# timfpark/heatmap

Hardware: AMD Instinct MI355X
Metric: points binned/sec (whole node, zooms 0-18) + % HBM roofline at 1/2/4/8 GPU (higher is better)
Workload: dtype f64

## Files before the change

heatmap_amd/csrc/hm_api.cpp:

```cpp
#include <hip/hip_runtime.h>
#include <stdio.h>
#include <stdlib.h>
#include <string.h>

#include <math.h>

#include <algorithm>
#include <chrono>
#include <vector>

#include "hm_genkey.h"
#include "hm_ctx.h"

namespace {

struct Level {
    int zc;
    int dbits;
    uint32_t nparents;
    uint64_t nchildren;
    uint32_t count = 0;
    uint32_t items = 0;
    bool out16 = false;
};
// ... 82 lines not shown
    case HM_E_WIDE: return "a routed count needs 64 bits (route again with count_bytes = 8)";
    case HM_E_HIP: return "HIP runtime error";
    case HM_E_NOMEM: return "device allocation failed";
    default: return "unknown status";
    }
}

int hm_ctx_create(hm_ctx** out, int device, void* stream)
{
    if (!out) return HM_E_ARG;
    *out = nullptr;
    int n = 0;
    if (hipGetDeviceCount(&n) != hipSuccess || n <= device || device < 0) {
        (void)hipGetLastError();
        fprintf(stderr, "heatmap_amd: no HIP device %d (found %d); there is no CPU fallback\n", device, n);
        return HM_E_HIP;
    }
    HIPCHK(hipSetDevice(device));
    hm_ctx* c = new hm_ctx();
    c->device = device;
    c->stream = (hipStream_t)stream;
    c->bufs.resize(B_COUNT);
    for (int i = 0; i < HM_NEV; i++) c->ev[i] = nullptr;
    c->spread_min_keys = HM_SPREAD_MIN_KEYS;
    if (const char* e = getenv("HM_SPREAD_MIN_KEYS")) c->spread_min_keys = atof(e);
    c->spread_min_cold = HM_SPREAD_MIN_COLD;
    if (const char* e = getenv("HM_SPREAD_MIN_COLD")) c->spread_min_cold = atof(e);
    c->rs_big_min = HM_RS_BIG;
    if (const char* e = getenv("HM_RS_BIG_MIN")) c->rs_big_min = (uint64_t)atoll(e);
    if (const char* e = getenv("HM_HOT")) c->hot = atoi(e);
    if (const char* e = getenv("HM_HOT_MID")) c->hot_mid = atoi(e);
    if (const char* e = getenv("HM_HOT_INV_SHARE")) c->hot_inv_share = atof(e);
    if (const char* e = getenv("HM_HOT_MIN_KEYS")) c->hot_min_keys = atof(e);
    if (const char* e = getenv("HM_RUN_SHARD_BITS")) c->run_shard_bits = atoi(e);
    if (const char* e = getenv("HM_SAMPLE_LOG2")) c->sample_log2 = std::min(30, std::max(8, atoi(e)));
    if (const char* e = getenv("HM_DEBUG_L1")) c->debug_l1 = atoi(e);
    if (const char* e = getenv("HM_STAGE_TIMING")) c->stage_timing = atoi(e);
    if (const char* e = getenv("HM_CONTIG")) c->contig = atoi(e);
    if (const char* e = getenv("HM_TA_MIN")) c->ta_min = (uint32_t)std::max(1024, std::min((int)HM_TA, atoi(e)));
    if (const char* e = getenv("HM_TA_ITEMS")) c->ta_items = (uint32_t)std::max(1, atoi(e));
    int st = HM_OK;
    if (hipMalloc(&c->state, ST_COUNT * sizeof(unsigned long long)) != hipSuccess) {
        c->state = nullptr;
        st = HM_E_NOMEM;
    } else if (hipHostMalloc(&c->host_state, 4 * ST_COUNT * sizeof(unsigned long long)) != hipSuccess) {
        c->host_state = nullptr;
        st = HM_E_NOMEM;
    } else if (hipHostMalloc(&c->host_aux, (2 + 2 * HM_L1_SHARDS) * HM_D1 * sizeof(uint32_t)) != hipSuccess) {
        c->host_aux = nullptr;
        st = HM_E_NOMEM;
    }
    for (int i = 0; i < HM_NEV && st == HM_OK; i++)
        if (hipEventCreate(&c->ev[i]) != hipSuccess) {
            c->ev[i] = nullptr;
            st = HM_E_HIP;
        }
    if (st != HM_OK) {
        (void)hipGetLastError();
        hm_ctx_destroy(c);
        return st;
    }
    *out = c;
    return HM_OK;
}

int hm_ctx_set_stream(hm_ctx* c, void* stream)
// ... 9 lines not shown
    double prev;
    if (!strcmp(name, "HM_SPREAD_MIN_KEYS")) {
        prev = c->spread_min_keys;
        c->spread_min_keys = value;
    } else if (!strcmp(name, "HM_SPREAD_MIN_COLD")) {
        prev = c->spread_min_cold;
        c->spread_min_cold = value;
    } else if (!strcmp(name, "HM_CONTIG")) {
        prev = c->contig;
        c->contig = value != 0;
    } else if (!strcmp(name, "HM_STAGE_TIMING")) {
        prev = c->stage_timing;
        c->stage_timing = value != 0;
    } else if (!strcmp(name, "HM_SAMPLE_LOG2")) {
        if (!(value >= 8 && value <= 30)) return HM_E_ARG;
        prev = c->sample_log2;
        c->sample_log2 = (int)value;
    } else if (!strcmp(name, "HM_RS_BIG_MIN")) {
        prev = (double)c->rs_big_min;
        c->rs_big_min = (uint64_t)(value < 0 ? 0 : value);
    } else if (!strcmp(name, "HM_HOT")) {
        prev = c->hot;
        c->hot = value != 0;
    } else if (!strcmp(name, "HM_HOT_MID")) {
        prev = c->hot_mid;
        c->hot_mid = value != 0;
    } else if (!strcmp(name, "HM_HOT_INV_SHARE")) {
        if (!(value >= 1)) return HM_E_ARG;
        prev = c->hot_inv_share;
        c->hot_inv_share = value;
    } else if (!strcmp(name, "HM_HOT_MIN_KEYS")) {
        prev = c->hot_min_keys;
        c->hot_min_keys = value;
    } else if (!strcmp(name, "HM_RUN_SHARD_BITS")) {
        if (value > 5) return HM_E_ARG;
        prev = c->run_shard_bits;
        c->run_shard_bits = value < 0 ? -1 : (int)value;
    } else if (!strcmp(name, "HM_TA_MIN")) {
        const uint32_t v = (value >= 1024 && value <= (double)HM_TA) ? (uint32_t)value : 0u;
        if (!v || (double)v != value || (v & (v - 1))) return HM_E_ARG;
        prev = c->ta_min;
        c->ta_min = v;
    } else if (!strcmp(name, "HM_TA_ITEMS")) {
        if (!(value >= 1 && value <= 4294967295.0)) return HM_E_ARG;
        prev = c->ta_items;
        c->ta_items = (uint32_t)value;
    } else {
        return HM_E_ARG;
    }
    if (old) *old = prev;
    return HM_OK;
}

int hm_ctx_destroy(hm_ctx* c)
{
    if (!c) return HM_OK;
    (void)hipSetDevice(c->device);
    for (auto& b : c->bufs)
        if (b.p) (void)hipFree(b.p);
    if (c->state) (void)hipFree(c->state);
    if (c->host_state) (void)hipHostFree(c->host_state);
    if (c->host_aux) (void)hipHostFree(c->host_aux);
    for (int i = 0; i < HM_NEV; i++)
        if (c->ev[i]) (void)hipEventDestroy(c->ev[i]);
    delete c;
    return HM_OK;
// ... 3 lines not shown
{
    if (!c) return HM_E_ARG;
    if (index) *index = c->last_err_index;
    if (kind) *kind = c->last_err_kind;
    return HM_OK;
}

int hm_last_stats(hm_ctx* c, int64_t* slow_points, double* stage_us, int n_stages)
{
    if (!c) return HM_E_ARG;
    if (slow_points) *slow_points = c->last_slow;
    for (int i = 0; i < n_stages && i < 9; i++) stage_us[i] = c->stage_us[i];
    if (n_stages > 7) stage_us[7] = (double)c->last_levels;
    return HM_OK;
}

}

void ctx_copy_tuning(hm_ctx* d, const hm_ctx* c)
{
    d->spread_min_keys = c->spread_min_keys;
    d->spread_min_cold = c->spread_min_cold;
    d->sample_log2 = c->sample_log2;
    d->debug_l1 = c->debug_l1;
    d->stage_timing = c->stage_timing;
    d->contig = c->contig;
    d->ta_min = c->ta_min;
    d->ta_items = c->ta_items;
    d->rs_big_min = c->rs_big_min;
    d->hot = c->hot;
    d->hot_mid = c->hot_mid;
    d->hot_inv_share = c->hot_inv_share;
    d->hot_min_keys = c->hot_min_keys;
    d->run_shard_bits = c->run_shard_bits;
}

static int reset_state(hm_ctx* ctx)
{
    HIPCHK(hipMemsetAsync(ctx->state, 0, ST_COUNT * sizeof(unsigned long long), ctx->stream));
    HIPCHK(hipMemsetAsync(ctx->state + ST_ERR, 0xFF, sizeof(unsigned long long), ctx->stream));
    return HM_OK;
}

static int read_state(hm_ctx* ctx)
{
    HIPCHK(hipMemcpyAsync(ctx->host_state, ctx->state, ST_COUNT * sizeof(unsigned long long), hipMemcpyDeviceToHost,
                          ctx->stream));
    HIPCHK(hm_sync(ctx->stream));
    return HM_OK;
}

static int take_error(hm_ctx* ctx)
{
    const unsigned long long e = ctx->host_state[ST_ERR];
    ctx->last_slow = (int64_t)ctx->host_state[ST_SLOW];
    if (e == ~0ull) {
        ctx->last_err_index = -1;
        ctx->last_err_kind = HM_OK;
        return HM_OK;
    }
    ctx->last_err_index = (int64_t)(e >> 8);
    ctx->last_err_kind = (int)(e & 0xFF);
    return ctx->last_err_kind;
}

extern "C" int hm_project(hm_ctx* ctx, const double* lat, const double* lon, int64_t n, int zoom, int64_t* row,
// ... 465 lines not shown
    hand.slot_k ^= 1;
    return HM_OK;
}

int CountCall::level1()
{
    int st;
    if ((st = begin_level(0))) return st;
    Level1Work w;
    if ((st = level1_setup(w))) return st;
    if ((st = level1_size(w))) return st;
    if ((st = level1_bucket_args(w))) return st;
    if ((st = level1_run(w))) return st;
    return level1_finish(w);
}

int CountCall::level1_setup(Level1Work& w)
{
    const Level& V = lv[0];
    HmFill f1;
    memset(&f1, 0, sizeof(f1));
    hm_fill_add(f1, ctx->state + 1, 0, (ST_COUNT - 1) * sizeof(unsigned long long));
    hm_fill_add(f1, ctx->state + ST_ERR, 0xFF, sizeof(unsigned long long));
    static_assert(ST_ERR == 0, "error word first");
    w.F = 1 << V.dbits;
    uint32_t* fill;
    ENSURE(B_L1_FILL, FS * 4, fill);
    ENSURE(B_L1_RBASE, FS * 4, w.rbase);
    ENSURE(B_L1_RCAP, FS * 4, w.rcap);
    ENSURE(B_L1_HIST, HM_D1 * 4, w.hist);
    ENSURE(B_L1_SMASK, HM_D1, w.smask);
    uint32_t* const hist = w.hist;
    uint4* l1slot = nullptr;
    if (!from_tiles) ENSURE(B_L1_SLOT, (size_t)FS * sizeof(uint4), l1slot);
    hot_mid = ctx->hot && ctx->hot_mid && L == 3 && zs[1] <= 11 && zs[0] == HM_Z1 && n > 0 && V.dbits == 2 * HM_Z1;
    hot_on = hot_mid || (ctx->hot && L == 2 && zb <= 11 && zs[0] == HM_Z1 && n > 0 && V.dbits == 2 * HM_Z1);
    hz = hot_mid ? zs[1] : zb;
    uint32_t* redo_idx = nullptr;
    w.redo_rows = w.redo_cols = nullptr;
    if (!from_tiles) {
        ENSURE(B_REDO_IDX, redo_cap * sizeof(uint32_t), redo_idx);
        ENSURE(B_REDO_ROWS, redo_cap * sizeof(int64_t), w.redo_rows);
        ENSURE(B_REDO_COLS, redo_cap * sizeof(int64_t), w.redo_cols);
    }
    HmPart1Args& a = w.a;
    memset(&a, 0, sizeof(a));
    a.lat = lat;
    a.lon = lon;
    a.rows_in = rows;
    a.cols_in = cols;
    a.keep = keep;
    a.n = n;
    a.Z = Z;
    a.dbits = V.dbits;
    a.restbits = 2 * (Z - zs[0]);
    a.fill = fill;
    a.rbase = w.rbase;
    a.rcap = w.rcap;
    a.smask = w.smask;
    a.l1slot = l1slot;
    a.overflow = ctx->state + ST_OVERFLOW;
    a.err_word = ctx->state + ST_ERR;
    a.x = xl;
    a.slow_count = ctx->state + ST_SLOW;
    a.redo_idx = redo_idx;
    a.redo_count = ctx->state + ST_REDO;
    a.redo_cap = redo_cap;
    const int slog = n < (1ll << 24) ? std::min(ctx->sample_log2, 16) : ctx->sample_log2;
    const uint64_t stride = w.stride = std::max<uint64_t>(1, (uint64_t)n >> slog);
    hm_fill_add(f1, hist, 0, HM_D1 * 4);
    hm_fill_add(f1, fill, 0, FS * 4);
    uint32_t* hot_counts = nullptr;
    uint32_t* hot_tiles = nullptr;
    uint32_t* hot_hash = nullptr;
    uint8_t* hot_parent = nullptr;
    uint32_t* hot_n = (uint32_t*)(ctx->state + ST_NHOT);
    if (hot_on) {
        ENSURE(B_HOT_COUNTS, (4ull << (2 * hz)), hot_counts);
        ENSURE(B_HOT, (HM_MAX_HOT + HM_HOT_SLOTS + 2 * HM_HOT_CAND + 1) * 4, hot_tiles);
        ENSURE(B_HOT_PARENT, HM_MAX_F1, hot_parent);
        hot_hash = hot_tiles + HM_MAX_HOT;
        hm_fill_add(f1, hot_counts, 0, 4ull << (2 * hz));
        hm_fill_add(f1, hot_hash + HM_HOT_SLOTS + 2 * HM_HOT_CAND, 0, 4);
        hm_fill_add(f1, hot_parent, 0, HM_MAX_F1);
        a.hot_z = hz;
        a.hot_bytes = hot_mid ? 4 : 2;
        a.hot_hash = hot_hash;
        a.hot_n = hot_n;
    } else {
        a.hot_z = -1;
    }
    hm_launch_fill(s, f1);
    if (n > 0) hm_launch_sample_digits(s, a, stride, hist, hot_counts);
// ... 1362 lines not shown
```

heatmap_amd/csrc/hm_ctx.h:

```cpp
#ifndef HM_CTX_H
#define HM_CTX_H

#include <hip/hip_runtime.h>

#include <vector>

#include "../../include/heatmap_amd.h"
#include "hm_pipeline.h"

#define HM_INTERNAL __attribute__((visibility("hidden")))

struct HM_INTERNAL Buf {
    void* p = nullptr;
    size_t cap = 0;
};

#define HM_NEV 12

#define HM_FALLBACK (-1)

struct hm_ctx {
    int device = 0;
    hipStream_t stream = nullptr;
    std::vector<Buf> bufs;
    unsigned long long* state = nullptr;
    unsigned long long* host_state = nullptr;
    int last_levels = 0;
    uint32_t* host_aux = nullptr;
    int64_t last_err_index = -1;
    int last_err_kind = 0;
    int64_t last_slow = 0;
    double stage_us[9] = {0};
    hipEvent_t ev[HM_NEV];
    double spread_min_keys = 0;
    double spread_min_cold = 0;
    int sample_log2 = 18;
    int debug_l1 = 0;
    int stage_timing = 1;
    int contig = 1;
    uint32_t ta_min = 16384;
    uint32_t ta_items = 128;
    uint64_t* tail_keys = nullptr;
    const unsigned long long* tail_state = nullptr;
    int tail_cb = 0;
    int tail_done = 0;
    uint64_t rs_big_min = 0;
    int hot = 1;
    int hot_mid = 1;
    double hot_inv_share = 4096;
    double hot_min_keys = 65536;
    int run_shard_bits = -1;
};

enum {
    ST_ERR = 0,
    ST_XCOUNT = 1,
    ST_SLOW = 2,
    ST_CURSOR = 3,
    ST_NSLOTS = 4,
    ST_REDO = 5,
    ST_REDO_OUT = 6,
    ST_XCURSOR = 7,
    ST_OVERFLOW = 8,
    ST_NHOT = 9,
    ST_L1TOTAL = 10,
    ST_LTOT = 12,
    ST_COUNT = 16
};

enum {
    B_KEYS_A, B_KEYS_B, B_RUNS_SH, B_FLAT_A, B_FLAT_B, B_EXCL_A, B_EXCL_B, B_CNT, B_SHOFF, B_NR, B_NRUNS,
    B_NKEYS, B_KEYBASE, B_VALS, B_PREFIX, B_PARTIAL, B_TOTAL, B_ROOT, B_REDO_IDX, B_REDO_ROWS, B_REDO_COLS,
    B_RUNBASE0,
    B_BK0 = B_RUNBASE0 + HM_MAX_LEVELS,
    B_CHILD0 = B_BK0 + HM_MAX_LEVELS * 8,
    B_TOT0 = B_CHILD0 + HM_MAX_LEVELS,
    B_SLOTS = B_TOT0 + HM_MAX_LEVELS + 1,
    B_SLOTBKT, B_GSLOTS, B_SPCODES, B_DESC0,
    B_X_ROW = B_DESC0 + HM_MAX_LEVELS, B_X_COL, B_X_IDX, B_GEN_KA, B_GEN_KB, B_GEN_FLAG, B_GEN_IDX, B_GEN_C,
    B_GEN_KHA, B_GEN_KHB, B_GEN_HIST, B_GEN_ORAND, B_GL_GRP,
    B_L1_FILL, B_L1_RBASE, B_L1_RCAP, B_L1_HIST, B_L1_SMASK,
    B_RT_CNT, B_RT_OFF, B_MG_TABLE, B_MG_STATE, B_SEG, B_RS_BIG,
    B_HOT, B_HOT_COUNTS, B_HOT_PARENT, B_D2B, B_MB_CNT, B_MB_OFF, B_MB_KEYS, B_MB_COUNTS, B_MB_CNT2, B_MB_OFF2,
// ... 43 lines not shown
```

heatmap_amd/csrc/hm_kernels.hip:

```cpp
#include <hip/hip_runtime.h>
#include "hm_genkey.h"
#include "hm_device.h"
#include "hm_project.h"
#include "hm_pipeline.h"
#define HM_STAMP_MODES(m) ((m) >= 1 && (m) <= 4)
#include "hm_stamps.h"
#include "hm_runs.h"

#define HM_YTAB_N (HM_YTAB_ROWS * HM_YTAB_STRIDE)
__constant__ double c_ytab[HM_YTAB_N] = HM_YTAB_INIT;

__device__ __forceinline__ void hm_load_ytab(double* tab)
{
    for (int i = threadIdx.x; i < HM_YTAB_N; i += blockDim.x) tab[i] = c_ytab[i];
}


__global__ __launch_bounds__(256) void k_project(const double* __restrict__ lat, const double* __restrict__ lon,
                                                 int64_t n, int zoom, int64_t* __restrict__ row,
                                                 int64_t* __restrict__ col, uint8_t* __restrict__ status,
                                                 unsigned long long* err_word, unsigned long long* slow_count)
{
    __shared__ double tab[HM_YTAB_N];
    hm_load_ytab(tab);
// ... 42 lines not shown
    return x;
}

#define HM_PIN16(x)                                                                                                   \
    "+v"(x[0]), "+v"(x[1]), "+v"(x[2]), "+v"(x[3]), "+v"(x[4]), "+v"(x[5]), "+v"(x[6]), "+v"(x[7]), "+v"(x[8]),       \
        "+v"(x[9]), "+v"(x[10]), "+v"(x[11]), "+v"(x[12]), "+v"(x[13]), "+v"(x[14]), "+v"(x[15])
template <int N>
__device__ __forceinline__ void hm_pin_all(uint32_t (&x)[N])
{
    if constexpr (N == 16) {
        asm volatile("" : HM_PIN16(x));
    } else {
#pragma unroll
        for (int k = 0; k < N; k++) asm volatile("" : "+v"(x[k]));
    }
}
template <int N>
__device__ __forceinline__ void hm_pin_all(uint32_t (&x)[N], uint32_t& y)
{
    if constexpr (N == 16) {
        asm volatile("" : HM_PIN16(x), "+v"(y));
    } else {
#pragma unroll
        for (int k = 0; k < N; k++) asm volatile("" : "+v"(x[k]));
        asm volatile("" : "+v"(y));
    }
}

typedef double hm_d2v __attribute__((ext_vector_type(2)));
__device__ __forceinline__ double2 hm_stream_load2(const double2* p)
{
    const hm_d2v v = __builtin_nontemporal_load((const hm_d2v*)p);
    return make_double2(v.x, v.y);
}

__device__ __forceinline__ uint32_t hm_hot_find(const uint2* tab, uint32_t rs, uint32_t cs)
{
    const uint2 e = tab[hm_hot_bucket(rs, cs)];
    const uint32_t tk = rs << HM_HOT_TAG;
    return min(e.x ^ tk, e.y ^ tk);
}


template <typename OutT, int MODE, bool FULL>
__global__ __launch_bounds__(HM_P1_THREADS, HM_P1_WAVES) void k_project_partition(HmPart1Args a)
{
    __shared__ uint32_t cur[HM_D1 + 64];
    __shared__ __attribute__((aligned(16))) OutT stage[HM_T1 + 64];
    __shared__ __attribute__((aligned(8))) uint16_t sdig[HM_T1 + 64];
    __shared__ unsigned long long scr[HM_P1_THREADS / 64 + 1];
    __shared__ double tab[HM_YTAB_N];
    constexpr bool HSEP = sizeof(OutT) * HM_T1 < HM_HOT_SLOTS * 4;
    constexpr bool RSEP = sizeof(uint16_t) * HM_T1 < HM_D1 * sizeof(uint2);
    __shared__ __attribute__((aligned(16))) uint32_t hsep[HSEP ? HM_HOT_SLOTS : 4];
    __shared__ __attribute__((aligned(8))) uint2 rsep[RSEP ? HM_D1 : 1];
    static_assert(sizeof(double) * HM_YTAB_N >= HM_D1 * 4, "dbase lives in the polynomial table");
    uint4* const hsh4 = HSEP ? (uint4*)hsep : (uint4*)stage;
    uint32_t* const dbase = (uint32_t*)tab;
    uint2* const rinfo = RSEP ? rsep : (uint2*)sdig;
    constexpr bool FROM_TILES = MODE == 1;
    const int tid = threadIdx.x;
    const int F = 1 << a.dbits;
    const uint32_t H = a.hot_z >= 0 ? *a.hot_n : 0u;
    const int64_t base = (a.tile0 + (int64_t)blockIdx.x) * HM_T1;
    const int64_t n = (FROM_TILES && a.n_dev) ? min((int64_t)*a.n_dev, a.n) : a.n;
    if (base >= n) return;
// ... 305 lines not shown
#endif
#define HM_L1_SLOTS (HM_MAX_HOT + HM_MAX_F1)
#define HM_L1_CW 1600
static_assert(HM_L1_CW >= HM_L1_SLOTS + 64 && HM_L1_CW % 64 == 0, "count and delta words pair as read2st64");
static_assert(HM_L1_SLOTS % HM_P1_THREADS == 0, "slots per thread");

#ifndef HM_L1_WAVES
#define HM_L1_WAVES 4
#endif

__device__ __forceinline__ uint32_t hm_l1_slot_digit(uint32_t sl, int wd)
{
    if (sl < HM_MAX_HOT) return HM_MAX_F1 + sl;
    const uint32_t u = sl - HM_MAX_HOT, m = (1u << wd) - 1u;
    return HM_SKEW_CUR ? ((u & ~m) | ((u - ((u >> wd) << 3)) & m)) : u;
}
__device__ __forceinline__ bool hm_l1_slot_live(uint32_t sl, uint32_t H, uint32_t F)
{
    return sl < HM_MAX_HOT ? sl < H : (sl - HM_MAX_HOT) < F;
}

__global__ __launch_bounds__(256) void k_l1_slots(HmPart1Args a, uint4* __restrict__ tab)
{
    const uint32_t sl = blockIdx.x * 256u + threadIdx.x, b = blockIdx.y;
    if (sl >= HM_D1) return;
    const uint32_t H = a.hot_z >= 0 ? min(*a.hot_n, (uint32_t)HM_MAX_HOT) : 0u;
    uint4 e = make_uint4(0u, 0u, 0u, 0u);
    if (hm_l1_slot_live(sl, H, 1u << a.dbits)) {
        const uint32_t d = hm_l1_slot_digit(sl, a.dbits >> 1);
        const uint32_t i = hm_l1i(d, a.smask[d] != 0 ? b : 0u);
        e = make_uint4(a.rbase[i], a.rcap[i], i, 0u);
    }
    tab[b * HM_D1 + sl] = e;
}

void hm_launch_l1_slots(hipStream_t s, const HmPart1Args& a)
{
    static_assert(HM_D1 == HM_MAX_HOT + HM_MAX_F1, "the table's rows are k_l1_fast's slots");
    hipLaunchKernelGGL(k_l1_slots, dim3((HM_D1 + 255) / 256, HM_L1_SHARDS), dim3(256), 0, s, a, (uint4*)a.l1slot);
}
template <typename OutT, bool KEEP>
__global__ __launch_bounds__(HM_P1_THREADS) __attribute__((amdgpu_waves_per_eu(HM_L1_WAVES, HM_L1_WAVES))) void
k_l1_fast(HmPart1Args a)
{
    __shared__ __attribute__((aligned(16))) uint2 ent[HM_T1 + 64];
    __shared__ uint32_t cw[2 * HM_L1_CW];
    __shared__ uint32_t scr[HM_P1_THREADS / 64 + 1];
    __shared__ uint32_t s_over;
    constexpr int YROWS = HM_YTAB_ROWS + 1;
    constexpr int YN = YROWS * HM_YTAB_STRIDE;
    static_assert(sizeof(double) * YN <= 16384 && HM_HOT_SLOTS * 4 <= 16384, "tables fit the stage");
    double* const tab = (double*)ent;
    uint2* const hot2 = (uint2*)((char*)ent + 16384);
    const int tid = threadIdx.x;
    const uint32_t H = a.hot_z >= 0 ? *a.hot_n : 0u;
    const int64_t base = (a.tile0 + (int64_t)blockIdx.x) * HM_T1;
    HM_STAMP_M(4, 0);
    const double scale = hm_exp2i(a.Z);
    const double nscale = -scale, hscale = 0.5 * scale;
    const double kz = HM_INV360 * scale;
    const double c180 = 180.0 * kz;
    const double ghalf = 0.5 - HM_Y_EPS * scale;
    const double ghalf2 = 0.5 - scale * 0x1p-49;
    constexpr int PERD = HM_L1_SLOTS / HM_P1_THREADS;
    const int wd = a.dbits >> 1;
    uint32_t kp[HM_P1_PPT / 2];
    if (KEEP) {
        const uint16_t* kp2 = (const uint16_t*)(a.keep + base);
#pragma unroll
        for (int k = 0; k < HM_P1_PPT / 2; k++) kp[k] = kp2[k * HM_P1_THREADS + tid];
    } else {
#pragma unroll
        for (int k = 0; k < HM_P1_PPT / 2; k++) kp[k] = 0x0101;
    }
    __builtin_amdgcn_sched_barrier(0);
    constexpr int TPT = (YN + HM_P1_THREADS - 1) / HM_P1_THREADS;
    double tv[TPT];
#pragma unroll
    for (int q = 0; q < TPT; q++) {
        const int i = q * HM_P1_THREADS + tid;
        tv[q] = i >= HM_YTAB_N ? __builtin_nan("") : c_ytab[i];
    }
    uint4 st[PERD];
    {
        const uint4* const row = a.l1slot + (blockIdx.x & (HM_L1_SHARDS - 1)) * HM_L1_SLOTS;
#pragma unroll
        for (int q = 0; q < PERD; q++) st[q] = row[q * HM_P1_THREADS + tid];
    }
    constexpr int HV = HM_HOT_SLOTS / 4 / HM_P1_THREADS;
    uint4 hv[HV];
    static_assert(HM_HOT_SLOTS <= HM_D1 * HM_L1_SHARDS, "the stand-in array holds a hot table's bytes");
    const uint4* const hsrc = H ? (const uint4*)a.hot_hash : (const uint4*)a.rbase;
#pragma unroll
    for (int j = 0; j < HV; j++) {
        const uint4 v = hsrc[j * HM_P1_THREADS + tid];
        hv[j] = make_uint4(v.x, v.y, v.z, v.w);
    }
    __builtin_amdgcn_sched_barrier(0);
    double2 la[HM_P1_PPT / 2], lo[HM_P1_PPT / 2];
    {
        const double2* lat2 = (const double2*)(a.lat + base);
        const double2* lon2 = (const double2*)(a.lon + base);
#pragma unroll
        for (int k = 0; k < HM_P1_PPT / 2; k++) {
            la[k] = hm_stream_load2(lat2 + k * HM_P1_THREADS + tid);
            lo[k] = hm_stream_load2(lon2 + k * HM_P1_THREADS + tid);
        }
    }
    for (int i = tid; i < HM_L1_CW; i += HM_P1_THREADS) cw[i] = 0;
    if (tid == 0) s_over = 0;
    if (H) {
#pragma unroll
        for (int j = 0; j < HV; j++) ((uint4*)hot2)[j * HM_P1_THREADS + tid] = hv[j];
    }
#pragma unroll
    for (int q = 0; q < TPT; q++) {
        const int i = q * HM_P1_THREADS + tid;
        if (i < YN) tab[i] = tv[q];
    }
    hm_lds_barrier();
    HM_STAMP_M(4, 1);
    const int hb = a.restbits >> 1;
    const uint32_t lowm = (1u << hb) - 1u;
    const uint32_t keym = (uint32_t)((1ull << (2 * hb)) - 1ull);
    const uint32_t wm = (1u << wd) - 1u;
    const int hs = a.hot_z >= 0 ? a.Z - a.hot_z : 0;
    const uint32_t dummy = HM_L1_SLOTS + (uint32_t)hm_lane();
    uint32_t slot[HM_P1_PPT], key[HM_P1_PPT];
    uint32_t redo = 0;
#pragma unroll
    for (int k = 0; k < HM_P1_PPT; k++) {
        const double pa = (k & 1) ? la[k >> 1].y : la[k >> 1].x;
        const double po = (k & 1) ? lo[k >> 1].y : lo[k >> 1].x;
        uint32_t r, c;
        const bool ok = hm_project_l1(pa, po, nscale, hscale, kz, c180, ghalf, ghalf2, tab, &r, &c);
        const bool kept = ((kp[k >> 1] >> (8 * (k & 1))) & 0xFFu) != 0;
        redo |= (uint32_t)!ok << k;
        const uint32_t rd = r >> hb, cd = c >> hb;
        const uint32_t rdw = (rd << wd) + HM_MAX_HOT;
        uint32_t sl = HM_SKEW_CUR ? (((cd + (rd << 3)) & wm) | rdw) : (cd | rdw);
        if (H) sl = min(hm_hot_find(hot2, r >> hs, c >> hs), sl);
        key[k] = ((r << hb) | (c & lowm)) & keym;
        slot[k] = (ok & kept) ? sl : dummy;
        asm volatile("" : "+v"(slot[k]), "+v"(key[k]));
        __builtin_amdgcn_sched_barrier(0);
    }
    HM_STAMP_M(4, 2);
    if (__builtin_amdgcn_ballot_w64(redo != 0)) {
#pragma unroll
        for (int k = 0; k < HM_P1_PPT; k++) {
            const bool rd = (redo >> k) & 1u;
            const uint64_t m = __builtin_amdgcn_ballot_w64(rd);
            if (m) {
                uint64_t b = 0;
                if (hm_lane() == __ffsll((unsigned long long)m) - 1) b = atomicAdd(a.redo_count, (unsigned long long)__popcll(m));
                b = __shfl(b, __ffsll((unsigned long long)m) - 1, 64);
                const uint64_t q = b + hm_mbcnt(m);
                if (rd && q < a.redo_cap)
                    a.redo_idx[q] = (uint32_t)(base + 2 * ((int64_t)(k >> 1) * HM_P1_THREADS + tid) + (k & 1));
            }
        }
        const uint32_t ws = hm_wave_sum((uint32_t)__popc(redo));
        if (hm_lane() == 0 && ws) atomicAdd(a.slow_count, (unsigned long long)ws);
    }
    uint32_t rank[HM_P1_PPT];
    uint32_t merged = 0;
#pragma unroll
    for (int k = 0; k < HM_P1_PPT; k++) {
        const uint32_t k0 = __builtin_amdgcn_readfirstlane(slot[k]);
        const uint64_t m = __builtin_amdgcn_ballot_w64(slot[k] == k0);
        const uint32_t pm = (uint32_t)__builtin_popcount((uint32_t)m) + (uint32_t)__builtin_popcount((uint32_t)(m >> 32));
        uint32_t idx = slot[k], inc = 1u;
        if (pm >= HM_L1_MERGE_MIN) {
            merged |= 1u << k;
            const bool in = (m >> hm_lane()) & 1ull;
            idx = (in && hm_lane() != 0) ? dummy : idx;
            inc = hm_lane() == 0 ? pm : inc;
        }
        rank[k] = atomicAdd(&cw[idx], inc);
    }
    if (merged) {
#pragma unroll
        for (int k = 0; k < HM_P1_PPT; k++)
            if ((merged >> k) & 1u) {
                const uint32_t k0 = __builtin_amdgcn_readfirstlane(slot[k]);
                const uint64_t m = __builtin_amdgcn_ballot_w64(slot[k] == k0);
                const uint32_t r0 = __builtin_amdgcn_readfirstlane(rank[k]);
                if ((m >> hm_lane()) & 1ull) rank[k] = r0 + hm_mbcnt(m);
            }
    }
    hm_lds_barrier();
    HM_STAMP_M(4, 3);
    uint32_t cnt[PERD], gpos[PERD];
#pragma unroll
    for (int q = 0; q < PERD; q++) {
        const uint32_t sl = q * HM_P1_THREADS + tid;
        cnt[q] = cw[sl];
        gpos[q] = 0;
        if (cnt[q]) gpos[q] = atomicAdd(&a.fill[st[q].z], cnt[q]);
    }
    constexpr int QH = HM_MAX_HOT / HM_P1_THREADS;
    static_assert(HM_MAX_HOT % HM_P1_THREADS == 0 && QH >= 1 && QH < PERD, "slots q < QH are the hot tiles");
    uint32_t csum = 0, hsum = 0;
#pragma unroll
    for (int q = 0; q < PERD; q++) (q < QH ? hsum : csum) += cnt[q];
    uint32_t tot2;
    const uint32_t pre = hm_block_excl_scan<HM_P1_THREADS, true>(csum | (hsum << 16), scr, &tot2);
    const uint32_t C = tot2 & 0xFFFFu, total = C + (tot2 >> 16);
    uint32_t offq[PERD];
    {
        uint32_t oc = pre & 0xFFFFu, oh = C + (pre >> 16);
#pragma unroll
        for (int q = 0; q < PERD; q++) {
            offq[q] = q < QH ? oh : oc;
            (q < QH ? oh : oc) += cnt[q];
        }
    }
    bool over = false;
    auto deltas = [&]() {
#pragma unroll
        for (int q = 0; q < PERD; q++) {
            const uint32_t sl = q * HM_P1_THREADS + tid;
            const uint32_t rc = st[q].y, rb = st[q].x;
            const bool fits = (uint64_t)gpos[q] + cnt[q] <= (uint64_t)rc;
            over |= cnt[q] && !fits;
            cw[HM_L1_CW + sl] = (fits ? rb + gpos[q] : 0xFFF00000u) - offq[q];
        }
        if (over) {
            atomicOr(a.overflow, 1ull);
            s_over = 1;
        }
    };
#pragma unroll
    for (int q = 0; q < PERD; q++) {
        const uint32_t sl = q * HM_P1_THREADS + tid;
        cw[sl] = offq[q];
    }
    hm_lds_barrier();
    HM_STAMP_M(4, 4);
#pragma unroll
    for (int k = 0; k < HM_P1_PPT; k++) {
        const uint32_t o = cw[slot[k]];
        const uint32_t pos = slot[k] < HM_L1_SLOTS ? o + rank[k] : HM_T1 + (uint32_t)hm_lane();
        ent[pos] = make_uint2(key[k], slot[k]);
    }
    deltas();
    hm_lds_barrier();
    HM_STAMP_M(4, 5);
    char* const outb = (char*)a.keys_out;
    char* const houtb = (char*)a.keys_hot;
    const uint32_t hm = (1u << hs) - 1u;
    auto put_cold = [&](uint2 e) { *(OutT*)(outb + (uint64_t)e.y * sizeof(OutT)) = (OutT)e.x; };
    const bool hot32 = a.hot_bytes == 4;
    auto put_hot = [&](uint2 e) {
        const uint32_t hk = (((e.x >> hb) & hm) << hs) | (e.x & hm);
        if (hot32) *(uint32_t*)(houtb + (uint64_t)e.y * 4u) = hk;
        else *(uint16_t*)(houtb + (uint64_t)e.y * 2u) = (uint16_t)hk;
    };
    uint2 e[HM_P1_PPT];
    uint32_t sov;
    uint32_t dl[HM_P1_PPT];
#pragma unroll
    for (int j = 0; j < HM_P1_PPT; j++) {
        e[j] = ent[j * HM_P1_THREADS + tid];
        dl[j] = e[j].y;
    }
    hm_pin_all(dl);
#pragma unroll
    for (int j = 0; j < HM_P1_PPT; j++) dl[j] = cw[HM_L1_CW + min(dl[j], (uint32_t)(HM_L1_CW - 1))];
    sov = s_over;
    hm_pin_all(dl, sov);
    sov = __builtin_amdgcn_readfirstlane(sov);
#pragma unroll
    for (int j = 0; j < HM_P1_PPT; j++) e[j].y = dl[j] + (uint32_t)(j * HM_P1_THREADS + tid);
    const uint32_t wofs = (uint32_t)tid & ~63u;
    if (!sov) {
#pragma unroll
        for (int j = 0; j < HM_P1_PPT; j++) {
            const uint32_t wb = __builtin_amdgcn_readfirstlane(j * HM_P1_THREADS + wofs);
            const uint32_t i = j * HM_P1_THREADS + tid;
            if (wb + 64 <= C) {
                put_cold(e[j]);
            } else if (wb >= C && wb + 64 <= total) {
                put_hot(e[j]);
            } else if (wb < total) {
                if (i < C) put_cold(e[j]);
                else if (i < total) put_hot(e[j]);
            }
        }
    } else {
#pragma unroll
        for (int j = 0; j < HM_P1_PPT; j++) {
            const uint32_t i = j * HM_P1_THREADS + tid;
            if (i < total && e[j].y < 0xFFF00000u) {
                if (i < C) put_cold(e[j]);
                else put_hot(e[j]);
            }
        }
    }
    HM_STAMP_M(4, 6);
}

#define HM_SAMPLE_HSLOTS 4096
template <bool FROM_TILES, bool HOT>
__global__ __launch_bounds__(256) void k_sample_digits(HmPart1Args a, uint64_t stride_pts, uint32_t* hist,
                                                       uint32_t* hot_counts)
{
    __shared__ uint32_t h[HM_MAX_F1 + 64];
    __shared__ double tab[HM_YTAB_N];
    __shared__ uint32_t hk[HOT ? HM_SAMPLE_HSLOTS : 1], hc[HOT ? HM_SAMPLE_HSLOTS : 1];
    const int F = 1 << a.dbits;
    for (int i = threadIdx.x; i < F; i += 256) h[i] = 0;
    if (HOT)
        for (int i = threadIdx.x; i < HM_SAMPLE_HSLOTS; i += 256) {
            hk[i] = HM_HOT_EMPTY;
            hc[i] = 0;
        }
    if (!FROM_TILES) hm_load_ytab(tab);
    __syncthreads();
    uint32_t hlost = 0;
    const double scale = hm_exp2i(a.Z);
    const double kz = HM_INV360 * scale;
    const uint32_t lim = 1u << a.Z;
    const int hb = a.restbits >> 1, wd = a.dbits >> 1;
    const uint64_t m = (uint64_t)(a.n + stride_pts - 1) / stride_pts;
    const uint64_t m_up = (m + 63) & ~63ull;
    const uint64_t step = (uint64_t)gridDim.x * 256;
    for (uint64_t j = (uint64_t)blockIdx.x * 256 + threadIdx.x; j < m_up; j += step) {
        const uint64_t i = j * stride_pts;
// ... 1601 lines not shown
```

heatmap_amd/csrc/hm_pipeline.h:

```cpp
#pragma once
#include <hip/hip_runtime.h>
#include <stdint.h>

#include "hm_top_select.h"

#ifndef HM_P1_THREADS
#define HM_P1_THREADS 512
#endif
#ifndef HM_P1_PPT
#define HM_P1_PPT 16
#endif
#define HM_T1 (HM_P1_THREADS * HM_P1_PPT)
#ifndef HM_P1_GROUP
#define HM_P1_GROUP 4
#endif
#ifndef HM_P1_ILP
#define HM_P1_ILP 1
#endif
#ifndef HM_P1_WAVES
#define HM_P1_WAVES 1
#endif
#define HM_L1_SHARDS 8
#ifndef HM_L1_SHARD_TILES
#define HM_L1_SHARD_TILES 16
#endif
#define HM_L1_ZERO_SAMPLES 24
#define HM_Z1 5
#define HM_MAX_F1 1024
#ifndef HM_MAX_HOT
#define HM_MAX_HOT 512
#endif
#define HM_HOT_LIMIT HM_MAX_HOT
#define HM_D1 (HM_MAX_F1 + HM_MAX_HOT)
#define HM_HOT_WAYS 2
#define HM_HOT_SLOTS 4096
#define HM_HOT_BUCKETS (HM_HOT_SLOTS / HM_HOT_WAYS)
#define HM_HOT_BBITS 11
#define HM_HOT_TAG 16
#define HM_HOT_MULT 0x9E3779u
#define HM_HOT_CAND 4096
#define HM_HOT_EMPTY 0xFFFFFFFFu
static_assert(HM_MAX_HOT <= 1024 && (HM_MAX_HOT & 255) == 0, "hot tiles");
__host__ __device__ inline uint32_t hm_hot_bucket(uint32_t rs, uint32_t cs)
{
#if defined(__HIP_DEVICE_COMPILE__)
    return (__umul24(rs, HM_HOT_MULT) + cs) & (HM_HOT_BUCKETS - 1u);
#else
    return (rs * HM_HOT_MULT + cs) & (HM_HOT_BUCKETS - 1u);
#endif
}
static_assert(HM_HOT_MULT < (1u << 24), "24-bit hash multiplier");
static_assert(HM_HOT_BUCKETS == 1 << HM_HOT_BBITS, "hot-tile table");
__host__ __device__ inline uint32_t hm_l1i(uint32_t d, uint32_t sh) { return sh * HM_D1 + d; }
#ifndef HM_PN_THREADS
#define HM_PN_THREADS 1024
#endif
#ifndef HM_TN
#define HM_TN 8192
#endif
#ifndef HM_FR_THREADS
#define HM_FR_THREADS 1024
#endif
#ifndef HM_FR_GROUP
#define HM_FR_GROUP 4
#endif
#ifndef HM_LEVEL_ZOOMS
#define HM_LEVEL_ZOOMS 6
#endif
#define HM_MAX_FN 4096
#define HM_MAX_SHARDS 32
#ifndef HM_RUN_SHARD_BITS
#define HM_RUN_SHARD_BITS 4
#endif
#define HM_AG_THREADS 1024
#define HM_AG_CELLS 16384
#define HM_AG_LG 7
#ifndef HM_TA
#define HM_TA (1u << 18)
#endif
#ifndef HM_SP_MAX
#define HM_SP_MAX 512
#endif
#ifndef HM_SPW_MAX
#define HM_SPW_MAX HM_SP_MAX
#endif
#ifndef HM_SPW_SPLIT
// ... 77 lines not shown
    uint64_t cap;
    unsigned long long* count;
};

struct HmCompactOut {
    uint32_t* nkeys;
    uint32_t* nruns;
    uint32_t* rbase;
    uint32_t* keybase;
    uint32_t* item_begin;
    uint32_t* digit;
    uint64_t* coord;
};

struct HmPart1Args {
    const double* lat;
    const double* lon;
    const int64_t* rows_in;
    const int64_t* cols_in;
    const uint8_t* keep;
    int64_t n;
    int64_t tile0;
    const unsigned long long* n_dev;
    int Z, dbits, restbits;
    uint32_t* redo_idx;
    unsigned long long* redo_count;
    uint64_t redo_cap;
    void* keys_out;
    uint32_t* fill;
    const uint32_t* rbase;
    const uint32_t* rcap;
    const uint8_t* smask;
    const uint4* l1slot;
    unsigned long long* overflow;
    unsigned long long* err_word;
    HmExotic x;
    unsigned long long* slow_count;
    int hot_z;
    int hot_bytes;
    void* keys_hot;
    const uint32_t* hot_hash;
    const uint32_t* hot_n;
};

struct HmHotArgs {
    uint32_t* counts;
    int zb, z1;
    uint32_t thresh;
    uint32_t* tiles;
    uint32_t* hist;
    uint8_t* hotparent;
    uint32_t* n;
    uint32_t* hash;
    uint32_t* cand;
};

struct HmHotRunArgs {
    const uint32_t* tiles;
    const uint32_t* n;
    int zb, z1, dbits;
    int zp;
    const uint32_t* c2b;
    const uint32_t* fill;
    const uint32_t* rbase;
    const uint32_t* d2b;
    uint64_t* nr;
// ... 695 lines not shown
```

Baseline: 198.2 billion.

## Use buffer loads/stores with 32-bit offsets and prebuilt hot-table image in L1 kernel

```diff
diff --git a/heatmap_amd/csrc/hm_api.cpp b/heatmap_amd/csrc/hm_api.cpp
--- a/heatmap_amd/csrc/hm_api.cpp
+++ b/heatmap_amd/csrc/hm_api.cpp
@@ -138,6 +138,7 @@
     if (const char* e = getenv("HM_HOT_MID")) c->hot_mid = atoi(e);
     if (const char* e = getenv("HM_HOT_INV_SHARE")) c->hot_inv_share = atof(e);
     if (const char* e = getenv("HM_HOT_MIN_KEYS")) c->hot_min_keys = atof(e);
+    if (const char* e = getenv("HM_L1_OFF32_LIMIT")) c->l1_off32_limit = (uint64_t)std::max(0.0, atof(e));
     if (const char* e = getenv("HM_RUN_SHARD_BITS")) c->run_shard_bits = atoi(e);
     if (const char* e = getenv("HM_SAMPLE_LOG2")) c->sample_log2 = std::min(30, std::max(8, atoi(e)));
     if (const char* e = getenv("HM_DEBUG_L1")) c->debug_l1 = atoi(e);
@@ -213,6 +214,10 @@
     } else if (!strcmp(name, "HM_HOT_MIN_KEYS")) {
         prev = c->hot_min_keys;
         c->hot_min_keys = value;
+    } else if (!strcmp(name, "HM_L1_OFF32_LIMIT")) {
+        if (!(value >= 0 && value <= (double)HM_L1_OFF32_LIMIT)) return HM_E_ARG;
+        prev = (double)c->l1_off32_limit;
+        c->l1_off32_limit = (uint64_t)value;
     } else if (!strcmp(name, "HM_RUN_SHARD_BITS")) {
         if (value > 5) return HM_E_ARG;
         prev = c->run_shard_bits;
@@ -282,6 +287,7 @@
     d->hot_mid = c->hot_mid;
     d->hot_inv_share = c->hot_inv_share;
     d->hot_min_keys = c->hot_min_keys;
+    d->l1_off32_limit = c->l1_off32_limit;
     d->run_shard_bits = c->run_shard_bits;
 }
 
@@ -813,7 +819,7 @@
     ENSURE(B_L1_SMASK, HM_D1, w.smask);
     uint32_t* const hist = w.hist;
     uint4* l1slot = nullptr;
-    if (!from_tiles) ENSURE(B_L1_SLOT, (size_t)FS * sizeof(uint4), l1slot);
+    if (!from_tiles) ENSURE(B_L1_SLOT, (size_t)FS * sizeof(uint4) + HM_L1_IMG_WORDS * 4, l1slot);
     hot_mid = ctx->hot && ctx->hot_mid && L == 3 && zs[1] <= 11 && zs[0] == HM_Z1 && n > 0 && V.dbits == 2 * HM_Z1;
     hot_on = hot_mid || (ctx->hot && L == 2 && zb <= 11 && zs[0] == HM_Z1 && n > 0 && V.dbits == 2 * HM_Z1);
     hz = hot_mid ? zs[1] : zb;
@@ -840,6 +846,9 @@
     a.rcap = w.rcap;
     a.smask = w.smask;
     a.l1slot = l1slot;
+    a.l1img = l1slot ? (const uint32_t*)(l1slot + FS) : nullptr;
+    a.out_bytes = V.out16 ? 2 : 4;
+    a.off32_limit = ctx->l1_off32_limit;
     a.overflow = ctx->state + ST_OVERFLOW;
     a.err_word = ctx->state + ST_ERR;
     a.x = xl;
diff --git a/heatmap_amd/csrc/hm_ctx.h b/heatmap_amd/csrc/hm_ctx.h
--- a/heatmap_amd/csrc/hm_ctx.h
+++ b/heatmap_amd/csrc/hm_ctx.h
@@ -49,6 +49,7 @@
     int hot_mid = 1;
     double hot_inv_share = 4096;
     double hot_min_keys = 65536;
+    uint64_t l1_off32_limit = 1ull << 32;
     int run_shard_bits = -1;
 };
 
diff --git a/heatmap_amd/csrc/hm_kernels.hip b/heatmap_amd/csrc/hm_kernels.hip
--- a/heatmap_amd/csrc/hm_kernels.hip
+++ b/heatmap_amd/csrc/hm_kernels.hip
@@ -98,6 +98,14 @@
 {
     const hm_d2v v = __builtin_nontemporal_load((const hm_d2v*)p);
     return make_double2(v.x, v.y);
+}
+
+typedef uint32_t hm_u4v __attribute__((ext_vector_type(4)));
+typedef uint32_t hm_u2v __attribute__((ext_vector_type(2)));
+#define HM_BUF_NT 2
+__device__ __forceinline__ __amdgpu_buffer_rsrc_t hm_buf(const void* p, uint32_t bytes)
+{
+    return __builtin_amdgcn_make_buffer_rsrc((void*)p, 0, (int)bytes, 0x00020000);
 }
 
 __device__ __forceinline__ uint32_t hm_hot_find(const uint2* tab, uint32_t rs, uint32_t cs)
@@ -469,6 +477,23 @@
         e = make_uint4(a.rbase[i], a.rcap[i], i, 0u);
     }
     tab[b * HM_D1 + sl] = e;
+    if (b == 0) {
+        uint32_t* const img = (uint32_t*)a.l1img;
+        for (uint32_t i = sl; i < HM_HOT_SLOTS; i += HM_D1) {
+            const uint32_t v = H ? a.hot_hash[i] : HM_HOT_EMPTY;
+            img[i] = v == HM_HOT_EMPTY ? v : (v & ~0xFFFFu) | ((v & 0xFFFFu) << 2);
+        }
+        if (sl == 0) {
+            const uint32_t ic = hm_l1i((1u << a.dbits) - 1u, HM_L1_SHARDS - 1);
+            const uint32_t ih = hm_l1i(HM_MAX_F1 + (H ? H - 1u : 0u), HM_L1_SHARDS - 1);
+            const uint64_t cend = (uint64_t)a.rbase[ic] + a.rcap[ic];
+            const uint64_t hend = H ? (uint64_t)a.rbase[ih] + a.rcap[ih] : 0ull;
+            img[HM_HOT_SLOTS] = H;
+            img[HM_HOT_SLOTS + 1] = hm_l1_off32_bytes(cend, (uint32_t)a.out_bytes, a.off32_limit);
+            img[HM_HOT_SLOTS + 2] = H ? hm_l1_off32_bytes(hend, (uint32_t)a.hot_bytes, a.off32_limit) : 0u;
+            img[HM_HOT_SLOTS + 3] = 0u;
+        }
+    }
 }
 
 void hm_launch_l1_slots(hipStream_t s, const HmPart1Args& a)
@@ -480,17 +505,24 @@
 __global__ __launch_bounds__(HM_P1_THREADS) __attribute__((amdgpu_waves_per_eu(HM_L1_WAVES, HM_L1_WAVES))) void
 k_l1_fast(HmPart1Args a)
 {
-    __shared__ __attribute__((aligned(16))) uint2 ent[HM_T1 + 64];
-    __shared__ uint32_t cw[2 * HM_L1_CW];
-    __shared__ uint32_t scr[HM_P1_THREADS / 64 + 1];
-    __shared__ uint32_t s_over;
+    struct Lds {
+        uint32_t cw[2 * HM_L1_CW];
+        uint32_t scr[HM_P1_THREADS / 64 + 1];
+        uint32_t over;
+        __attribute__((aligned(16))) uint2 ent[HM_T1 + 64];
+    };
+    __shared__ Lds lds;
+    static_assert(offsetof(Lds, cw) == 0 && sizeof(lds.cw) < 65536, "the slot words' offsets fit the offset field");
+    uint2* const ent = lds.ent;
+    uint32_t* const cw = lds.cw;
+    uint32_t* const scr = lds.scr;
+    uint32_t& s_over = lds.over;
     constexpr int YROWS = HM_YTAB_ROWS + 1;
     constexpr int YN = YROWS * HM_YTAB_STRIDE;
     static_assert(sizeof(double) * YN <= 16384 && HM_HOT_SLOTS * 4 <= 16384, "tables fit the stage");
     double* const tab = (double*)ent;
     uint2* const hot2 = (uint2*)((char*)ent + 16384);
     const int tid = threadIdx.x;
-    const uint32_t H = a.hot_z >= 0 ? *a.hot_n : 0u;
     const int64_t base = (a.tile0 + (int64_t)blockIdx.x) * HM_T1;
     HM_STAMP_M(4, 0);
     const double scale = hm_exp2i(a.Z);
@@ -503,58 +535,63 @@
     const int wd = a.dbits >> 1;
     uint32_t kp[HM_P1_PPT / 2];
     if (KEEP) {
-        const uint16_t* kp2 = (const uint16_t*)(a.keep + base);
-#pragma unroll
-        for (int k = 0; k < HM_P1_PPT / 2; k++) kp[k] = kp2[k * HM_P1_THREADS + tid];
+        const __amdgpu_buffer_rsrc_t rk = hm_buf(a.keep + base, HM_T1);
+#pragma unroll
+        for (int k = 0; k < HM_P1_PPT / 2; k++)
+            kp[k] = (uint16_t)__builtin_amdgcn_raw_buffer_load_b16(rk, (uint32_t)tid * 2u, k * HM_P1_THREADS * 2, 0);
     } else {
 #pragma unroll
         for (int k = 0; k < HM_P1_PPT / 2; k++) kp[k] = 0x0101;
     }
     __builtin_amdgcn_sched_barrier(0);
     constexpr int TPT = (YN + HM_P1_THREADS - 1) / HM_P1_THREADS;
-    double tv[TPT];
+    const uint32_t o16 = (uint32_t)tid * 16u;
+    hm_u2v tv[TPT];
+    {
+        const __amdgpu_buffer_rsrc_t ry = hm_buf(c_ytab, HM_YTAB_N * sizeof(double));
+#pragma unroll
+        for (int q = 0; q < TPT; q++)
+            tv[q] = __builtin_amdgcn_raw_buffer_load_b64(ry, (uint32_t)tid * 8u, q * HM_P1_THREADS * 8, 0);
+    }
+    hm_u4v st[PERD];
+    {
+        const __amdgpu_buffer_rsrc_t rs =
+            hm_buf(a.l1slot + (blockIdx.x & (HM_L1_SHARDS - 1)) * HM_L1_SLOTS, HM_L1_SLOTS * sizeof(uint4));
+#pragma unroll
+        for (int q = 0; q < PERD; q++) st[q] = __builtin_amdgcn_raw_buffer_load_b128(rs, o16, q * HM_P1_THREADS * 16, 0);
+    }
+    constexpr int HV = HM_HOT_SLOTS / 4 / HM_P1_THREADS;
+    hm_u4v hv[HV];
+    hm_u4v hd;
+    {
+        const __amdgpu_buffer_rsrc_t rh = hm_buf(a.l1img, HM_L1_IMG_WORDS * 4);
+#pragma unroll
+        for (int j = 0; j < HV; j++) hv[j] = __builtin_amdgcn_raw_buffer_load_b128(rh, o16, j * HM_P1_THREADS * 16, 0);
+        hd = __builtin_amdgcn_raw_buffer_load_b128(rh, 0u, HM_HOT_SLOTS * 4, 0);
+    }
+    __builtin_amdgcn_sched_barrier(0);
+    hm_u4v la[HM_P1_PPT / 2], lo[HM_P1_PPT / 2];
+    {
+        const __amdgpu_buffer_rsrc_t rla = hm_buf(a.lat + base, HM_T1 * sizeof(double));
+        const __amdgpu_buffer_rsrc_t rlo = hm_buf(a.lon + base, HM_T1 * sizeof(double));
+#pragma unroll
+        for (int k = 0; k < HM_P1_PPT / 2; k++) {
+            la[k] = __builtin_amdgcn_raw_buffer_load_b128(rla, o16, k * HM_P1_THREADS * 16, HM_BUF_NT);
+            lo[k] = __builtin_amdgcn_raw_buffer_load_b128(rlo, o16, k * HM_P1_THREADS * 16, HM_BUF_NT);
+        }
+    }
+    __builtin_amdgcn_sched_barrier(0);
+    for (int i = tid; i < HM_L1_CW; i += HM_P1_THREADS) cw[i] = 0;
+    if (tid == 0) s_over = 0;
+#pragma unroll
+    for (int j = 0; j < HV; j++) ((hm_u4v*)hot2)[j * HM_P1_THREADS + tid] = hv[j];
 #pragma unroll
     for (int q = 0; q < TPT; q++) {
         const int i = q * HM_P1_THREADS + tid;
-        tv[q] = i >= HM_YTAB_N ? __builtin_nan("") : c_ytab[i];
-    }
-    uint4 st[PERD];
-    {
-        const uint4* const row = a.l1slot + (blockIdx.x & (HM_L1_SHARDS - 1)) * HM_L1_SLOTS;
-#pragma unroll
-        for (int q = 0; q < PERD; q++) st[q] = row[q * HM_P1_THREADS + tid];
-    }
-    constexpr int HV = HM_HOT_SLOTS / 4 / HM_P1_THREADS;
-    uint4 hv[HV];
-    static_assert(HM_HOT_SLOTS <= HM_D1 * HM_L1_SHARDS, "the stand-in array holds a hot table's bytes");
-    const uint4* const hsrc = H ? (const uint4*)a.hot_hash : (const uint4*)a.rbase;
-#pragma unroll
-    for (int j = 0; j < HV; j++) {
-        const uint4 v = hsrc[j * HM_P1_THREADS + tid];
-        hv[j] = make_uint4(v.x, v.y, v.z, v.w);
-    }
-    __builtin_amdgcn_sched_barrier(0);
-    double2 la[HM_P1_PPT / 2], lo[HM_P1_PPT / 2];
-    {
-        const double2* lat2 = (const double2*)(a.lat + base);
-        const double2* lon2 = (const double2*)(a.lon + base);
-#pragma unroll
-        for (int k = 0; k < HM_P1_PPT / 2; k++) {
-            la[k] = hm_stream_load2(lat2 + k * HM_P1_THREADS + tid);
-            lo[k] = hm_stream_load2(lon2 + k * HM_P1_THREADS + tid);
-        }
-    }
-    for (int i = tid; i < HM_L1_CW; i += HM_P1_THREADS) cw[i] = 0;
-    if (tid == 0) s_over = 0;
-    if (H) {
-#pragma unroll
-        for (int j = 0; j < HV; j++) ((uint4*)hot2)[j * HM_P1_THREADS + tid] = hv[j];
-    }
-#pragma unroll
-    for (int q = 0; q < TPT; q++) {
-        const int i = q * HM_P1_THREADS + tid;
-        if (i < YN) tab[i] = tv[q];
-    }
+        if (i < YN) tab[i] = i >= HM_YTAB_N ? __builtin_nan("") : __builtin_bit_cast(double, tv[q]);
+    }
+    const uint32_t H = __builtin_amdgcn_readfirstlane(hd.x);
+    const uint32_t cold32 = __builtin_amdgcn_readfirstlane(hd.y), hot32b = __builtin_amdgcn_readfirstlane(hd.z);
     hm_lds_barrier();
     HM_STAMP_M(4, 1);
     const int hb = a.restbits >> 1;
@@ -562,20 +599,20 @@
     const uint32_t keym = (uint32_t)((1ull << (2 * hb)) - 1ull);
     const uint32_t wm = (1u << wd) - 1u;
     const int hs = a.hot_z >= 0 ? a.Z - a.hot_z : 0;
-    const uint32_t dummy = HM_L1_SLOTS + (uint32_t)hm_lane();
+    const uint32_t dummy = (HM_L1_SLOTS + (uint32_t)hm_lane()) * 4u;
     uint32_t slot[HM_P1_PPT], key[HM_P1_PPT];
     uint32_t redo = 0;
 #pragma unroll
     for (int k = 0; k < HM_P1_PPT; k++) {
-        const double pa = (k & 1) ? la[k >> 1].y : la[k >> 1].x;
-        const double po = (k & 1) ? lo[k >> 1].y : lo[k >> 1].x;
+        const double pa = __builtin_bit_cast(double, (k & 1) ? la[k >> 1].zw : la[k >> 1].xy);
+        const double po = __builtin_bit_cast(double, (k & 1) ? lo[k >> 1].zw : lo[k >> 1].xy);
         uint32_t r, c;
         const bool ok = hm_project_l1(pa, po, nscale, hscale, kz, c180, ghalf, ghalf2, tab, &r, &c);
         const bool kept = ((kp[k >> 1] >> (8 * (k & 1))) & 0xFFu) != 0;
         redo |= (uint32_t)!ok << k;
         const uint32_t rd = r >> hb, cd = c >> hb;
-        const uint32_t rdw = (rd << wd) + HM_MAX_HOT;
-        uint32_t sl = HM_SKEW_CUR ? (((cd + (rd << 3)) & wm) | rdw) : (cd | rdw);
+        const uint32_t rdw = (rd << (wd + 2)) + HM_MAX_HOT * 4u;
+        uint32_t sl = HM_SKEW_CUR ? ((((cd + (rd << 3)) & wm) << 2) | rdw) : ((cd << 2) | rdw);
         if (H) sl = min(hm_hot_find(hot2, r >> hs, c >> hs), sl);
         key[k] = ((r << hb) | (c & lowm)) & keym;
         slot[k] = (ok & kept) ? sl : dummy;
@@ -614,7 +651,7 @@
             idx = (in && hm_lane() != 0) ? dummy : idx;
             inc = hm_lane() == 0 ? pm : inc;
         }
-        rank[k] = atomicAdd(&cw[idx], inc);
+        rank[k] = atomicAdd((uint32_t*)((char*)cw + idx), inc);
     }
     if (merged) {
 #pragma unroll
@@ -677,8 +714,8 @@
     HM_STAMP_M(4, 4);
 #pragma unroll
     for (int k = 0; k < HM_P1_PPT; k++) {
-        const uint32_t o = cw[slot[k]];
-        const uint32_t pos = slot[k] < HM_L1_SLOTS ? o + rank[k] : HM_T1 + (uint32_t)hm_lane();
+        const uint32_t o = *(const uint32_t*)((const char*)cw + slot[k]);
+        const uint32_t pos = slot[k] < HM_L1_SLOTS * 4u ? o + rank[k] : HM_T1 + (uint32_t)hm_lane();
         ent[pos] = make_uint2(key[k], slot[k]);
     }
     deltas();
@@ -687,12 +724,22 @@
     char* const outb = (char*)a.keys_out;
     char* const houtb = (char*)a.keys_hot;
     const uint32_t hm = (1u << hs) - 1u;
-    auto put_cold = [&](uint2 e) { *(OutT*)(outb + (uint64_t)e.y * sizeof(OutT)) = (OutT)e.x; };
+    const __amdgpu_buffer_rsrc_t rco = hm_buf(a.keys_out, cold32), rho = hm_buf(a.keys_hot, hot32b);
+    auto put_cold = [&](uint2 e, bool narrow) __attribute__((always_inline)) {
+        if (!narrow) *(OutT*)(outb + (uint64_t)e.y * sizeof(OutT)) = (OutT)e.x;
+        else if (sizeof(OutT) == 2) __builtin_amdgcn_raw_buffer_store_b16((uint16_t)e.x, rco, e.y << 1, 0, 0);
+        else __builtin_amdgcn_raw_buffer_store_b32(e.x, rco, e.y << 2, 0, 0);
+    };
     const bool hot32 = a.hot_bytes == 4;
-    auto put_hot = [&](uint2 e) {
-        const uint32_t hk = (((e.x >> hb) & hm) << hs) | (e.x & hm);
-        if (hot32) *(uint32_t*)(houtb + (uint64_t)e.y * 4u) = hk;
-        else *(uint16_t*)(houtb + (uint64_t)e.y * 2u) = (uint16_t)hk;
+    auto put_hot = [&](uint2 e, bool narrow) __attribute__((always_inline)) {
+        const uint32_t hk = ((e.x >> (hb - hs)) & (hm << hs)) | (e.x & hm);
+        if (hot32) {
+            if (narrow) __builtin_amdgcn_raw_buffer_store_b32(hk, rho, e.y << 2, 0, 0);
+            else *(uint32_t*)(houtb + (uint64_t)e.y * 4u) = hk;
+        } else {
+            if (narrow) __builtin_amdgcn_raw_buffer_store_b16((uint16_t)hk, rho, e.y << 1, 0, 0);
+            else *(uint16_t*)(houtb + (uint64_t)e.y * 2u) = (uint16_t)hk;
+        }
     };
     uint2 e[HM_P1_PPT];
     uint32_t sov;
@@ -704,34 +751,39 @@
     }
     hm_pin_all(dl);
 #pragma unroll
-    for (int j = 0; j < HM_P1_PPT; j++) dl[j] = cw[HM_L1_CW + min(dl[j], (uint32_t)(HM_L1_CW - 1))];
+    for (int j = 0; j < HM_P1_PPT; j++)
+        dl[j] = *(const uint32_t*)((const char*)cw + HM_L1_CW * 4u + min(dl[j], (uint32_t)(HM_L1_CW - 1) * 4u));
     sov = s_over;
     hm_pin_all(dl, sov);
     sov = __builtin_amdgcn_readfirstlane(sov);
 #pragma unroll
     for (int j = 0; j < HM_P1_PPT; j++) e[j].y = dl[j] + (uint32_t)(j * HM_P1_THREADS + tid);
     const uint32_t wofs = (uint32_t)tid & ~63u;
-    if (!sov) {
+    auto clean = [&](bool cn, bool hn) __attribute__((always_inline)) {
 #pragma unroll
         for (int j = 0; j < HM_P1_PPT; j++) {
             const uint32_t wb = __builtin_amdgcn_readfirstlane(j * HM_P1_THREADS + wofs);
             const uint32_t i = j * HM_P1_THREADS + tid;
             if (wb + 64 <= C) {
-                put_cold(e[j]);
+                put_cold(e[j], cn);
             } else if (wb >= C && wb + 64 <= total) {
-                put_hot(e[j]);
+                put_hot(e[j], hn);
             } else if (wb < total) {
-                if (i < C) put_cold(e[j]);
-                else if (i < total) put_hot(e[j]);
-            }
-        }
+                if (i < C) put_cold(e[j], cn);
+                else if (i < total) put_hot(e[j], hn);
+            }
+        }
+    };
+    if (!sov) {
+        if (cold32 && (hot32b || !H)) clean(true, true);
+        else clean(false, false);
     } else {
 #pragma unroll
         for (int j = 0; j < HM_P1_PPT; j++) {
             const uint32_t i = j * HM_P1_THREADS + tid;
             if (i < total && e[j].y < 0xFFF00000u) {
-                if (i < C) put_cold(e[j]);
-                else put_hot(e[j]);
+                if (i < C) put_cold(e[j], false);
+                else put_hot(e[j], false);
             }
         }
     }
diff --git a/heatmap_amd/csrc/hm_l1_offsets.h b/heatmap_amd/csrc/hm_l1_offsets.h
--- /dev/null
+++ b/heatmap_amd/csrc/hm_l1_offsets.h
@@ -0,0 +1,23 @@
+#ifndef HM_L1_OFFSETS_H
+#define HM_L1_OFFSETS_H
+
+#include <stdint.h>
+
+#if defined(__HIPCC__)
+#define HM_L1O_FN __host__ __device__ static inline
+#else
+#define HM_L1O_FN static inline
+#endif
+
+#define HM_L1_OFF32_LIMIT (1ull << 32)
+
+HM_L1O_FN int hm_l1_bytes_fit32(uint64_t bytes, uint64_t limit) { return bytes < limit; }
+
+HM_L1O_FN uint32_t hm_l1_off32_bytes(uint64_t positions, uint32_t key_bytes, uint64_t limit)
+{
+    const uint64_t bytes = positions * (uint64_t)key_bytes;
+    if (limit > HM_L1_OFF32_LIMIT) limit = HM_L1_OFF32_LIMIT;
+    return hm_l1_bytes_fit32(bytes, limit) ? (uint32_t)bytes : 0u;
+}
+
+#endif
diff --git a/heatmap_amd/csrc/hm_pipeline.h b/heatmap_amd/csrc/hm_pipeline.h
--- a/heatmap_amd/csrc/hm_pipeline.h
+++ b/heatmap_amd/csrc/hm_pipeline.h
@@ -3,6 +3,7 @@
 #include <stdint.h>
 
 #include "hm_top_select.h"
+#include "hm_l1_offsets.h"
 
 #ifndef HM_P1_THREADS
 #define HM_P1_THREADS 512
@@ -52,6 +53,7 @@
 static_assert(HM_HOT_MULT < (1u << 24), "24-bit hash multiplier");
 static_assert(HM_HOT_BUCKETS == 1 << HM_HOT_BBITS, "hot-tile table");
 __host__ __device__ inline uint32_t hm_l1i(uint32_t d, uint32_t sh) { return sh * HM_D1 + d; }
+#define HM_L1_IMG_WORDS (HM_HOT_SLOTS + 4)
 #ifndef HM_PN_THREADS
 #define HM_PN_THREADS 1024
 #endif
@@ -195,6 +197,9 @@
     const uint32_t* rcap;
     const uint8_t* smask;
     const uint4* l1slot;
+    const uint32_t* l1img;
+    int out_bytes;
+    uint64_t off32_limit;
     unsigned long long* overflow;
     unsigned long long* err_word;
     HmExotic x;
```

Result: no change. 198.1 billion (median of 2 runs) (-0.1%).
